# NVIDIA-Genomics-Research/GenomeWorks

Measured on AMD Instinct MI355X. Metric: cudapoa consensus GCUPS, 1024-window short-read batch (static band 256, 32 reads <= 1024 bp), higher is better.
Workload: dtype int16; 1 GPU; BASELINE configs[2]: cudapoa single-batch consensus, 1024 windows x 32 reads, backbone 960 bp, <=48 sub/24 ins/24 del, BatchConfig(1024,32,256,static_band), scores 8/-6/-8; windows_per_gpu=1024, cells_per_gpu=10990578176, parallelism=index-split x1

## Files before the change

### genomeworks_amd/csrc/poa_forward_moves.h

```cpp
#pragma once

namespace gwhip
{

constexpr int kKindShift = 60;
constexpr uint32_t kMoveHoriz = 1;

__device__ __forceinline__ uint32_t pk_mad_u16_vsv(uint32_t a, uint32_t s, uint32_t c)
{
    uint32_t d;
    asm("v_pk_mad_u16 %0, %1, %2, %3" : "=v"(d) : "v"(a), "s"(s), "v"(c));
    return d;
}
__device__ __forceinline__ uint32_t pk_mad_u16_vvs(uint32_t a, uint32_t b, uint32_t s)
{
    uint32_t d;
    asm("v_pk_mad_u16 %0, %1, %2, %3" : "=v"(d) : "v"(a), "v"(b), "s"(s));
    return d;
}
__device__ __forceinline__ void gstore_nt_u64(void* p, uint32_t lo, uint32_t hi)
{
    u32x2 v;
    v.x = lo; v.y = hi;
    __builtin_nontemporal_store(v, reinterpret_cast<u32x2*>(p));
}
__device__ __forceinline__ void gstore_u16_lane0_below(const void* vptr, uint32_t v)
{
    asm volatile("s_mov_b64 exec, 1\n\tglobal_store_short %0, %1, off offset:-2\n\ts_mov_b64 exec, -1" ::"v"(vptr), "v"(v) : "memory");
}

template <int MAXD = kPkMaxDist, bool TBRULES = false>
__device__ __forceinline__ int32_t classify_kinds(RowInfo<true>* rowinfo, int32_t graph_count, int lane, const uint64_t* xpred, int32_t dbg = 0)
{
    int32_t first_moved = graph_count + 1;
    for (int32_t r = 1 + lane; r <= graph_count; r += kWave)
    {
        RowInfo<true> ri  = rowinfo[r];
        const int32_t cnt = ri.cnt(), bs = ri.bs();
        uint64_t kind     = 4;
        const uint64_t xe  = (cnt > 3 && cnt <= 6 && xpred != nullptr) ? xpred[r & 255] : 0ull;
        const bool many_ok = cnt > 3 && cnt <= 6 && xpred_hit(xe, r, cnt) && !(dbg & (1 << 30));
        if (cnt >= 1 && (cnt <= 3 || many_ok))
        {
            bool ok    = true;
            int32_t d0 = 0, pbs0 = 0;
            for (int32_t k = 0; k < cnt; k++)
            {
                const int32_t p   = k < 3 ? ri.pred(k) : xpred_row(xe, k);
                const int32_t d   = r - p;
                const RowInfo<true> pri = rowinfo[p];
                const int32_t pbs = pri.bs();
                ok                = ok && d >= 1 && d <= MAXD && (bs - pbs) <= kPkGuardCols && (bs == 0 || pbs > 0);
                if constexpr (TBRULES) ok = ok && !(pri.cnt() == 0 && pbs > 0);
                if (k == 0) { d0 = d; pbs0 = pbs; }
            }
            if (ok) kind = cnt > 1 ? 3 : ((d0 == 1 && pbs0 == bs) ? 0 : ((d0 == 1 && bs - pbs0 == kCellsPerLane) ? 1 : 2));
        }
        if ((dbg & 1024) && kind <= 1) kind = 2;
        if ((dbg & 32768) && kind == 1) kind = 2;
        if ((dbg & 512) && (kind == 2 || kind == 3)) kind = 4;
        if ((dbg & 2048) && kind <= 1) kind = 4;
        ri.w       = (ri.w & ~(7ull << kKindShift)) | (kind << kKindShift);
        rowinfo[r] = ri;
        if (bs > 0) first_moved = min(first_moved, r);
    }
    for (int off = 32; off > 0; off >>= 1) first_moved = min(first_moved, __shfl_xor(first_moved, off));
    return __builtin_amdgcn_readfirstlane(first_moved);
}

constexpr uint64_t kRowScoresInHbm = 1ull << 63;
template <typename IdT>
__device__ __forceinline__ void mark_score_rows(const GraphView<IdT>& g, RowInfo<true>* rowinfo, int32_t graph_count, int lane, bool all_rows)
{
    auto mark = [&](int32_t row) {
        __hip_atomic_fetch_or(reinterpret_cast<uint32_t*>(&rowinfo[row].w) + 1, 0x80000000u, __ATOMIC_RELAXED, __HIP_MEMORY_SCOPE_WORKGROUP);
    };
    for (int32_t r = 1 + lane; r <= graph_count; r += kWave)
    {
        const uint64_t w    = rowinfo[r].w;
        const uint32_t kind = (uint32_t)(w >> kKindShift) & 7u;
        const int32_t cnt   = (int32_t)((w >> 8) & 0x3fu);
        const bool reads_or_recomputes = kind >= 4u || cnt > 3;
        if (reads_or_recomputes || ((w >> 14) & 1u) != 0 || all_rows) mark(r);
        if (reads_or_recomputes)
        {
            const int32_t node_id = cnt > 3 ? (int32_t)g.sorted_poa[r - 1] : 0;
            for (int32_t k = 0; k < cnt; k++)
                mark(k < 3 ? (int32_t)((w >> (24 + 12 * k)) & 0xfffu) : (int32_t)g.node_id_to_pos[g.incoming_edges[(int64_t)node_id * kEdges + k]] + 1);
        }
    }
    wave_sync();
}
__device__ __forceinline__ bool row_recompute_safe(uint64_t w)
{
    return ((uint32_t)(w >> kKindShift) & 7u) >= 4u || ((w >> 8) & 0x3fu) > 3u || ((w >> 15) & 0x1ffu) == 0u;
}

template <typename IdT, int BW>
__device__ __forceinline__ void banded_forward_moves(const GraphView<IdT>& g, RowInfo<true>* rowinfo, int32_t graph_count,
                                                     const uint8_t* lds_read, int16_t* scores, uint8_t* moves, uint8_t* ring,
                                                     const uint64_t* xpred, int32_t max_column, int32_t gap_score,
                                                     int32_t mismatch_score, int32_t match_score, int32_t dbg,
                                                     uint64_t* prof_acc, bool store_all = true)
{
    const bool abl       = (dbg & (1 << 14)) != 0;
    const bool st_scores = !(abl && (dbg & (1 << 26))), st_moves = !(abl && (dbg & (1 << 27)));
    const bool ab_ring = !(abl && (dbg & (1 << 20))), ab_guard = !(abl && (dbg & (1 << 19))), ab_scan = !(abl && (dbg & (1 << 18))),
               ab_moves = !(abl && (dbg & (1 << 17))), ab_rows = !(abl && (dbg & (1 << 16)));
    const int32_t ksel = prof_acc ? ((dbg >> 28) & 7) - 1 : -1;
    const bool kcount  = (dbg & (1 << 12)) != 0;
    uint64_t kacc      = 0;
    static_assert(BW == 128 || BW == 256, "band widths of the packed pass");
    constexpr int32_t band_width = BW;
    constexpr int32_t stride     = band_width + kRightPad;
    constexpr int kBandLanes     = BW / kCellsPerLane;
    const int lane               = threadIdx.x & (kWave - 1);
    const bool band_lane         = lane < kBandLanes;
    const int32_t lane4 = lane * 4, lane8 = lane * 8;
    const int32_t min_score = Limits<int16_t>::min / 2;

    const int32_t first_moved = classify_kinds(rowinfo, graph_count, lane, xpred, dbg);
    wave_sync();
    mark_score_rows<IdT>(g, rowinfo, graph_count, lane, store_all);

    const uint32_t MIN2   = pin_vgpr(pk_dup(min_score));
    const uint32_t SENT2  = pin_vgpr(pk_dup(kPkSentinel));
    const uint32_t GAP2   = pin_vgpr(pk_dup(gap_score));
    const uint32_t MAT2   = pin_vgpr(pk_dup(match_score));
    const uint32_t DIF2   = pin_vgpr(pk_dup(mismatch_score - match_score));
    const uint32_t ONE2   = pin_vgpr(0x00010001u);
    const uint32_t THREE2 = pin_vgpr(0x00030003u);
    const uint32_t NEG1   = pin_vgpr(0xffffffffu);
    const uint32_t K01 = pk_make((lane4 + 0) * gap_score, (lane4 + 1) * gap_score);
    const uint32_t K23 = pk_make((lane4 + 2) * gap_score, (lane4 + 3) * gap_score);
    const uint32_t ring_base = lds_addr(ring);
    const uint32_t read_base = lds_addr(lds_read);
    const uint32_t guard_off  = lane < 16 ? (uint32_t)(2 * BW) : (lane == 16 ? (uint32_t)-136 : (uint32_t)(120 - 16 * lane));
    const bool is_lane16      = lane == 16;
    const bool is_lane63      = lane == kBandLanes - 1;
    const uint32_t move_keep  = lane == 0 ? 0xffffff00u : 0xffffffffu;
    const uint32_t GUARD_HI_MIN = pin_vgpr(is_lane16 ? (((uint32_t)kPkSentinel & 0xffffu) | ((uint32_t)min_score << 16)) : pk_dup(kPkSentinel));
    const uint32_t S0X_MIN      = (uint32_t)min_score << 16;

    uint32_t P01 = pk_make((lane4 + 1) * gap_score, (lane4 + 2) * gap_score);
    uint32_t P23 = pk_make((lane4 + 3) * gap_score, (lane4 + 4) * gap_score);
    int32_t prev_rel0 = 0;
    uint32_t rd4  = lds_load_u32(read_base + lane4);
    uint32_t rd4n = lds_load_u32(read_base + lane4 + 4);
    uint32_t a1   = (uint32_t)lane8;
    uint32_t ga   = (a1 + guard_off) & (kPkSlotBytes - 1);
    uint8_t* const score_base = reinterpret_cast<uint8_t*>(scores) + lane8 + 2 * (1 + kRelShift);
    uint8_t* move_ptr  = moves + lane4 + (1 + kRelShift);

    if (BW == 256 || band_lane) lds_store_u64(ring_base + a1, P01, P23);
    lds_store_guard(ring_base + ga, SENT2, is_lane16 ? (((uint32_t)kPkSentinel & 0xffffu) | (0u << 16)) : SENT2);

    auto scan_row = [&](uint32_t s01, uint32_t s23, int32_t cu) {
        const uint32_t u01 = pk_sub(s01, K01), u23 = pk_sub(s23, K23);
        const uint32_t pm01 = pk_max(u01, (u01 << 16) | 0x8000u);
        const uint32_t pm23 = pk_max(u23, (u23 << 16) | 0x8000u);
        const int32_t m3    = (int32_t)pk_max(pm01, pm23) >> 16;
        const int32_t incl  = ab_scan ? wave_inclusive_max(m3) : m3;
        const int32_t excl  = max(wave_shr1(incl, cu), cu);
        const uint32_t ex2  = __builtin_amdgcn_perm((uint32_t)excl, (uint32_t)excl, 0x01000100u);
        const uint32_t m1b  = __builtin_amdgcn_perm(pm01, pm01, 0x03020302u);
        P01 = pk_add(pk_max(pm01, ex2), K01);
        P23 = pk_add(pk_max(pk_max(pm23, m1b), ex2), K23);
    };
    auto nz = [&](uint32_t a, uint32_t b) -> uint32_t { return pk_min_u16(pk_sub(a, b), ONE2); };
    auto costs = [&](uint32_t base4, uint32_t& c01, uint32_t& c23) {
        const uint32_t x   = rd4 ^ base4;
        const uint32_t x01 = __builtin_amdgcn_perm(0u, x, 0x0c010c00u);
        const uint32_t x23 = __builtin_amdgcn_perm(0u, x, 0x0c030c02u);
        c01 = pk_mad_u16(pk_min_u16(x01, ONE2), DIF2, MAT2);
        c23 = pk_mad_u16(pk_min_u16(x23, ONE2), DIF2, MAT2);
    };
    auto from_pred = [&](uint32_t s0x, uint32_t q01, uint32_t q23, uint32_t c01, uint32_t c23, uint32_t& D01, uint32_t& D23,
                         uint32_t& V01, uint32_t& V23) {
        D01 = pk_add(__builtin_amdgcn_alignbit(q01, s0x, 16), c01);
        D23 = pk_add(__builtin_amdgcn_alignbit(q23, q01, 16), c23);
        V01 = pk_add(q01, GAP2);
        V23 = pk_add(q23, GAP2);
    };
    auto store_row = [&](auto bs0_tag, int32_t r, int32_t rel0_val, uint32_t mv4, bool scores_to_hbm) {
        constexpr bool BS0 = decltype(bs0_tag)::value;
        move_ptr += stride;
        const uint32_t sbase = ring_base + (((uint32_t)r & (kPkSlots - 1)) * kPkSlotBytes);
        if (BS0 || __builtin_expect(scores_to_hbm, 0))
        {
            uint8_t* score_ptr = score_base + (uint32_t)r * (uint32_t)(stride * 2);
            if (st_scores && (BW == 256 || band_lane)) gstore_nt_u64(score_ptr, P01, P23);
            if constexpr (BS0) gstore_u16_lane0_below(score_ptr, (uint32_t)rel0_val);
        }
        if (ab_ring && (BW == 256 || band_lane)) lds_store_u64(sbase + a1, P01, P23);
        if constexpr (BS0)
        {
            const uint32_t rel0pk = ((uint32_t)kPkSentinel & 0xffffu) | ((uint32_t)rel0_val << 16);
            if (ab_guard) lds_store_guard(sbase + ga, SENT2, is_lane16 ? rel0pk : SENT2);
            prev_rel0 = rel0_val;
        }
        else if (ab_guard)
            lds_store_guard(sbase + ga, SENT2, GUARD_HI_MIN);
        if (st_moves && (BW == 256 || band_lane)) *reinterpret_cast<uint32_t*>(move_ptr) = mv4;
    };
    auto pack_moves = [&](uint32_t m01, uint32_t m23) -> uint32_t {
        return __builtin_amdgcn_perm(m23, m01, 0x06040200u) & move_keep;
    };

    auto general_row = [&](int32_t r, int32_t& prev_rel0_io) {
        const RowInfo<true> ri = uniform_row(rowinfo[r]);
        const int32_t bs       = ri.bs();
        const uint32_t base    = (uint32_t)ri.base();
        const int32_t prev_bs  = r > 1 ? uniform_row(rowinfo[r - 1]).bs() : 0;
        a1   = (uint32_t)(2 * bs + lane8) & (kPkSlotBytes - 1);
        ga   = (a1 + guard_off) & (kPkSlotBytes - 1);
        rd4  = lds_load_u32(read_base + bs + lane4);
        rd4n = lds_load_u32(read_base + bs + lane4 + 4);
        const int32_t pred_count = ri.cnt();
        const int32_t c          = bs + lane4;
        const int32_t cp0 = ((rd4 & 0xff) == base) ? match_score : mismatch_score;
        const int32_t cp1 = (((rd4 >> 8) & 0xff) == base) ? match_score : mismatch_score;
        const int32_t cp2 = (((rd4 >> 16) & 0xff) == base) ? match_score : mismatch_score;
        const int32_t cp3 = ((rd4 >> 24) == base) ? match_score : mismatch_score;
        const int32_t R0 = pk_lo(P01), R1 = pk_hi(P01), R2 = pk_lo(P23), R3 = pk_hi(P23);
        bool synced = false;
        auto from_regs = [&](int32_t& t0, int32_t& t1, int32_t& t2, int32_t& t3) {
            const int32_t q    = (bs - prev_bs) >> 2;
            const int32_t pend = min(prev_bs + band_width - kCellsPerLane, max_column);
            const int src      = lane + q;
            const int32_t from_left = __shfl(R3, src - 1);
            const int32_t S0        = (q == 0 && lane == 0) ? prev_rel0_io : from_left;
            const int32_t S1 = __shfl(R0, src), S2 = __shfl(R1, src), S3 = __shfl(R2, src), S4 = __shfl(R3, src);
            const bool valid = c <= pend;
            t0 = valid ? max(S0 + cp0, S1 + gap_score) : min_score;
            t1 = valid ? max(S1 + cp1, S2 + gap_score) : min_score;
            t2 = valid ? max(S2 + cp2, S3 + gap_score) : min_score;
            t3 = valid ? max(S3 + cp3, S4 + gap_score) : min_score;
        };
        auto from_hbm = [&](int32_t prow, int32_t& t0, int32_t& t1, int32_t& t2, int32_t& t3) {
            const int32_t pbs  = prow == 0 ? 0 : uniform_row(rowinfo[prow]).bs();
            const int32_t pend = min(pbs + band_width - kCellsPerLane, max_column);
            const bool valid   = !(c > pend || c < pbs);
            if (!synced) { wave_sync(); synced = true; }
            const int16_t* rowp = scores + (int64_t)prow * stride + (valid ? (c - pbs) : 0) + kRelShift;
            int32_t S0 = rowp[0];
            const Quad<int16_t> qd = *reinterpret_cast<const Quad<int16_t>*>(rowp + 1);
            const int32_t S1 = qd.v[0], S2 = qd.v[1], S3 = qd.v[2], S4 = qd.v[3];
            if (pbs > 0 && c == pbs) S0 = min_score;
            t0 = valid ? max(S0 + cp0, S1 + gap_score) : min_score;
            t1 = valid ? max(S1 + cp1, S2 + gap_score) : min_score;
            t2 = valid ? max(S2 + cp2, S3 + gap_score) : min_score;
            t3 = valid ? max(S3 + cp3, S4 + gap_score) : min_score;
        };
        auto rel0_of = [&](int32_t prow) -> int32_t {
            if (prow == r - 1) return prev_rel0_io;
            const int32_t pbs = prow == 0 ? 0 : uniform_row(rowinfo[prow]).bs();
            if (pbs > 0) return min_score;
            if (!synced) { wave_sync(); synced = true; }
            return wave_first((int32_t)scores[(int64_t)prow * stride + kRelShift]);
        };
        const int32_t node_id = (pred_count > 3) ? (int32_t)g.sorted_poa[r - 1] : 0;
        auto pred_row = [&](int32_t p) -> int32_t {
            if (pred_count == 0) return 0;
            if (p < 3) return ri.pred(p);
            return wave_first((int32_t)g.node_id_to_pos[g.incoming_edges[(int64_t)node_id * kEdges + p]] + 1);
        };
        int32_t fe = 0, rel0_val = min_score;
        if (pred_count == 0)
        {
            if (bs == 0) rel0_val = gap_score;
        }
        else
        {
            if (bs > kCellsPerLane && pred_count == 1)
                fe = min_score + gap_score;
            else
            {
                int32_t penalty = min_score;
                for (int32_t p = 0; p < pred_count; p++) penalty = max(penalty, rel0_of(pred_row(p)));
                fe = penalty + gap_score;
            }
            if (bs == 0) rel0_val = fe;
        }
        int32_t s0 = 0, s1 = 0, s2 = 0, s3 = 0;
        const int32_t np = max(pred_count, 1);
        for (int32_t p = 0; p < np; p++)
        {
            const int32_t prow = pred_row(p);
            int32_t t0, t1, t2, t3;
            if (prow == r - 1) from_regs(t0, t1, t2, t3);
            else from_hbm(prow, t0, t1, t2, t3);
            if (p == 0) { s0 = t0; s1 = t1; s2 = t2; s3 = t3; }
            else { s0 = max(s0, t0); s1 = max(s1, t1); s2 = max(s2, t2); s3 = max(s3, t3); }
        }
        scan_row(pk_make(s0, s1), pk_make(s2, s3), fe + gap_score);
        uint8_t* score_ptr = score_base + (uint32_t)r * (uint32_t)(stride * 2);
        move_ptr += stride;
        const uint32_t sbase  = ring_base + (((uint32_t)r & (kPkSlots - 1)) * kPkSlotBytes);
        const uint32_t rel0pk = ((uint32_t)kPkSentinel & 0xffffu) | ((uint32_t)rel0_val << 16);
        if (BW == 256 || band_lane)
        {
            *reinterpret_cast<uint2*>(score_ptr) = make_uint2(P01, P23);
            lds_store_u64(sbase + a1, P01, P23);
        }
        lds_store_guard(sbase + ga, SENT2, is_lane16 ? rel0pk : SENT2);
        if (bs == 0) gstore_u16_lane0_below(score_ptr, (uint32_t)rel0_val);
        if (BW == 256 || band_lane) *reinterpret_cast<uint32_t*>(move_ptr) = 0u;
        prev_rel0_io = rel0_val;
    };

    auto reg_row = [&](auto bs0_tag, auto moved_tag, int32_t r, uint32_t d0, uint32_t base4, bool scores_to_hbm) {
        constexpr bool BS0   = decltype(bs0_tag)::value;
        constexpr bool MOVED = decltype(moved_tag)::value;
        uint32_t s0x, q01, q23;
        if constexpr (!MOVED)
        {
            s0x = (uint32_t)wave_shr1((int32_t)P23, BS0 ? (int32_t)((uint32_t)prev_rel0 << 16) : (int32_t)S0X_MIN);
            q01 = P01; q23 = P23;
        }
        else
        {
            s0x  = P23;
            q01  = (uint32_t)wave_shl1((int32_t)P01, (int32_t)pk_dup(kPkSentinel));
            q23  = (uint32_t)wave_shl1((int32_t)P23, (int32_t)pk_dup(kPkSentinel));
            a1   = (a1 + 8) & (kPkSlotBytes - 1);
            ga   = (ga + 8) & (kPkSlotBytes - 1);
            rd4  = rd4n;
            rd4n = lds_load_u32(read_base + (((d0 >> 3) & 0x1ffu) << 2) + lane4 + 4);
        }
        int32_t cu = min_score + 2 * gap_score, rel0_val = min_score;
        if constexpr (BS0)
        {
            rel0_val = max(min_score, prev_rel0) + gap_score;
            cu       = rel0_val + gap_score;
        }
        uint32_t c01, c23, D01, D23, V01, V23;
        costs(base4, c01, c23);
        from_pred(s0x, q01, q23, c01, c23, D01, D23, V01, V23);
        uint32_t s01 = pk_max(D01, V01), s23 = pk_max(D23, V23);
        if constexpr (MOVED)
        {
            s01 = is_lane63 ? MIN2 : s01;
            s23 = is_lane63 ? MIN2 : s23;
        }
        scan_row(s01, s23, cu);
        const uint32_t m01 = pk_mad_u16(nz(P01, D01), pk_mad_u16(nz(P01, V01), NEG1, NEG1), THREE2);
        const uint32_t m23 = pk_mad_u16(nz(P23, D23), pk_mad_u16(nz(P23, V23), NEG1, NEG1), THREE2);
        uint32_t mv4 = ab_moves ? pack_moves(m01, m23) : 0u;
        if constexpr (MOVED) mv4 = is_lane63 ? 0u : mv4;
        store_row(bs0_tag, r, rel0_val, mv4, scores_to_hbm);
    };

    auto run_rows = [&](auto bs0_tag, int32_t r_from, int32_t r_to) {
        constexpr bool BS0 = decltype(bs0_tag)::value;
        int32_t r = r_from;
        while (r <= r_to)
        {
            const int32_t r0   = r;
            uint32_t D0v, D1v;
            {
                const int32_t rr    = min(r0 + lane, graph_count);
                const uint64_t w    = rowinfo[rr].w;
                const uint32_t kind = (uint32_t)(w >> kKindShift) & 7u;
                const uint32_t cnt  = (uint32_t)(w >> 8) & 0x3fu;
                const uint32_t bs4  = (uint32_t)(w >> 15) & 0x1ffu;
                const uint32_t p0 = (uint32_t)(w >> 24) & 0xfffu, p1 = (uint32_t)(w >> 36) & 0xfffu, p2 = (uint32_t)(w >> 48) & 0xfffu;
                const uint32_t slots = (p0 & 7u) | ((p1 & 7u) << 3) | ((p2 & 7u) << 6);
                const uint32_t dists = (((uint32_t)rr - p0) & 7u) | ((((uint32_t)rr - p1) & 7u) << 3) | ((((uint32_t)rr - p2) & 7u) << 6);
                D0v = kind | (bs4 << 3) | (slots << 12) | (dists << 21) | ((cnt <= 3 ? cnt : 0u) << 30);
                D1v = ((uint32_t)w & 0xffu) * 0x01010101u;
            }
            D0v = (r0 + lane <= r_to) ? D0v : 7u;
            const uint64_t need64 = BS0 ? ~0ull : __ballot((rowinfo[min(r0 + lane, graph_count)].w & kRowScoresInHbm) != 0);
            int32_t k      = 0;
            uint32_t d0    = (uint32_t)__builtin_amdgcn_readlane((int32_t)D0v, 0);
            uint32_t base4 = (uint32_t)__builtin_amdgcn_readlane((int32_t)D1v, 0);
            uint32_t kind  = d0 & 7u;
            auto advance = [&]() {
                r++;
                k++;
                const uint32_t nd = (uint32_t)__builtin_amdgcn_readlane((int32_t)D0v, k & (kWave - 1));
                base4 = (uint32_t)__builtin_amdgcn_readlane((int32_t)D1v, k & (kWave - 1));
                d0    = k == kWave ? 7u : nd;
                kind  = d0 & 7u;
            };
            for (;;)
            {
                const uint64_t t_k0 = ksel == 0 ? clock64() : 0;
                const int32_t r_k0  = r;
                while (kind == 0)
                {
                    reg_row(bs0_tag, std::false_type{}, r, d0, base4, ((need64 >> k) & 1ull) != 0);
                    advance();
                }
                if (ksel == 0) kacc += kcount ? (uint64_t)(r - r_k0) : clock64() - t_k0;
                if (kind == 7u) break;
                const int32_t kind_now = (int32_t)min(kind, 4u);
                const uint64_t t_kx    = ksel == kind_now ? clock64() : 0;
                const bool scores_to_hbm = ((need64 >> k) & 1ull) != 0;
                if (kind == 1)
                    reg_row(bs0_tag, std::true_type{}, r, d0, base4, scores_to_hbm);
                else if (kind <= 3)
                {
                    const uint32_t bs = ((d0 >> 3) & 0x1ffu) << 2;
                    a1 = (2u * bs + (uint32_t)lane8) & (kPkSlotBytes - 1);
                    ga = (a1 + guard_off) & (kPkSlotBytes - 1);
                    const uint32_t a0 = (a1 - 4) & (kPkSlotBytes - 1);
                    const uint32_t b0 = ring_base + (((d0 >> 12) & 7u) * kPkSlotBytes);
                    const uint32_t sent16 = (uint32_t)kPkSentinel & 0xffffu;
                    const uint32_t dd0 = (d0 >> 21) & 7u;
                    if (kind == 2)
                    {
                        const uint32_t x0 = lds_load_u32(b0 + a0);
                        const uint2 q0    = lds_load_u64(b0 + a1);
                        rd4  = lds_load_u32(read_base + bs + lane4);
                        rd4n = lds_load_u32(read_base + bs + lane4 + 4);
                        int32_t cu = min_score + 2 * gap_score, rel0_val = min_score;
                        if constexpr (BS0)
                        {
                            rel0_val = max(min_score, (int32_t)(int16_t)wave_first((int32_t)(lds_load_u32(b0 + kPkSlotBytes - 4) >> 16))) + gap_score;
                            cu       = rel0_val + gap_score;
                        }
                        uint32_t c01, c23, D01, D23, V01, V23;
                        costs(base4, c01, c23);
                        from_pred(x0, q0.x, q0.y, c01, c23, D01, D23, V01, V23);
                        const bool outside = (q0.x & 0xffffu) == sent16;
                        const uint32_t s01 = pk_max(D01, V01), s23 = pk_max(D23, V23);
                        scan_row(outside ? MIN2 : s01, outside ? MIN2 : s23, cu);
                        const uint32_t cD = pk_dup((int32_t)(2u * dd0 + 1u)), cV = pk_dup(1 - (int32_t)(2u * dd0));
                        const uint32_t m01 = pk_mad_u16_vvs(nz(P01, D01), pk_mad_u16_vsv(nz(P01, V01), cV, NEG1), cD);
                        const uint32_t m23 = pk_mad_u16_vvs(nz(P23, D23), pk_mad_u16_vsv(nz(P23, V23), cV, NEG1), cD);
                        const uint32_t mv4 = outside ? 0u : pack_moves(m01, m23);
                        store_row(bs0_tag, r, rel0_val, mv4, scores_to_hbm);
                    }
                    else
                    {
                        const uint32_t cnt3    = d0 >> 30;
                        const int32_t cnt      = cnt3 == 2 ? 2 : 3;
                        const uint32_t b1 = ring_base + (((d0 >> 15) & 7u) * kPkSlotBytes);
                        const uint32_t b2 = cnt > 2 ? ring_base + (((d0 >> 18) & 7u) * kPkSlotBytes) : b0;
                        const uint32_t dd1 = (d0 >> 24) & 7u, dd2 = (d0 >> 27) & 7u;
                        const uint32_t x0 = lds_load_u32(b0 + a0);
                        const uint2 q0    = lds_load_u64(b0 + a1);
                        const uint32_t x1 = lds_load_u32(b1 + a0);
                        const uint2 q1    = lds_load_u64(b1 + a1);
                        uint32_t x2 = 0;
                        uint2 q2 = make_uint2(0, 0);
                        if (cnt > 2)
                        {
                            x2 = lds_load_u32(b2 + a0);
                            q2 = lds_load_u64(b2 + a1);
                        }
                        rd4  = lds_load_u32(read_base + bs + lane4);
                        rd4n = lds_load_u32(read_base + bs + lane4 + 4);
                        int32_t fe = min_score + gap_score;
                        if constexpr (BS0)
                        {
                            int32_t pen = max(min_score, (int32_t)(int16_t)wave_first((int32_t)(lds_load_u32(b0 + kPkSlotBytes - 4) >> 16)));
                            pen = max(pen, (int32_t)(int16_t)wave_first((int32_t)(lds_load_u32(b1 + kPkSlotBytes - 4) >> 16)));
                            if (cnt > 2) pen = max(pen, (int32_t)(int16_t)wave_first((int32_t)(lds_load_u32(b2 + kPkSlotBytes - 4) >> 16)));
                            fe = pen + gap_score;
                        }
                        uint32_t c01, c23;
                        costs(base4, c01, c23);
                        uint32_t D0a, D0b, V0a, V0b, D1a, D1b, V1a, V1b;
                        from_pred(x0, q0.x, q0.y, c01, c23, D0a, D0b, V0a, V0b);
                        from_pred(x1, q1.x, q1.y, c01, c23, D1a, D1b, V1a, V1b);
                        const bool out0 = (q0.x & 0xffffu) == sent16, out1 = (q1.x & 0xffffu) == sent16;
                        bool undecided  = out0 | out1;
                        D0a = out0 ? MIN2 : D0a; D0b = out0 ? MIN2 : D0b; V0a = out0 ? MIN2 : V0a; V0b = out0 ? MIN2 : V0b;
                        D1a = out1 ? MIN2 : D1a; D1b = out1 ? MIN2 : D1b; V1a = out1 ? MIN2 : V1a; V1b = out1 ? MIN2 : V1b;
                        uint32_t bD01 = pk_max(D0a, D1a), bD23 = pk_max(D0b, D1b), bV01 = pk_max(V0a, V1a), bV23 = pk_max(V0b, V1b);
                        const uint32_t mD0 = pk_dup((int32_t)(2u * dd0 + 1u)), mV0 = pk_dup((int32_t)(2u * dd0));
                        const uint32_t E1  = pk_dup(2 * ((int32_t)dd1 - (int32_t)dd0));
                        uint32_t A01, A23, B01, B23;
                        if (cnt > 2)
                        {
                            uint32_t D2a, D2b, V2a, V2b;
                            from_pred(x2, q2.x, q2.y, c01, c23, D2a, D2b, V2a, V2b);
                            const bool out2 = (q2.x & 0xffffu) == sent16;
                            undecided       = undecided | out2;
                            D2a = out2 ? MIN2 : D2a; D2b = out2 ? MIN2 : D2b; V2a = out2 ? MIN2 : V2a; V2b = out2 ? MIN2 : V2b;
                            bD01 = pk_max(bD01, D2a); bD23 = pk_max(bD23, D2b); bV01 = pk_max(bV01, V2a); bV23 = pk_max(bV23, V2b);
                            const uint32_t E2  = pin_vgpr(pk_dup(2 * ((int32_t)dd2 - (int32_t)dd1)));
                            const uint32_t E1v = pin_vgpr(E1);
                            A01 = pk_mad_u16_vvs(nz(bD01, D0a), pk_mad_u16(nz(bD01, D1a), E2, E1v), mD0);
                            A23 = pk_mad_u16_vvs(nz(bD23, D0b), pk_mad_u16(nz(bD23, D1b), E2, E1v), mD0);
                            B01 = pk_mad_u16_vvs(nz(bV01, V0a), pk_mad_u16(nz(bV01, V1a), E2, E1v), mV0);
                            B23 = pk_mad_u16_vvs(nz(bV23, V0b), pk_mad_u16(nz(bV23, V1b), E2, E1v), mV0);
                        }
                        else
                        {
                            const uint32_t E1v = pin_vgpr(E1);
                            A01 = pk_mad_u16_vvs(nz(bD01, D0a), E1v, mD0); A23 = pk_mad_u16_vvs(nz(bD23, D0b), E1v, mD0);
                            B01 = pk_mad_u16_vvs(nz(bV01, V0a), E1v, mV0); B23 = pk_mad_u16_vvs(nz(bV23, V0b), E1v, mV0);
                        }
                        if (cnt3 == 0)
                        {
                            const uint64_t xe     = wave_first64(xpred[r & 255]);
                            const int32_t cnt_all = (int32_t)((xe >> 13) & 63u);
                            uint32_t xD01 = MIN2, xD23 = MIN2, xV01 = MIN2, xV23 = MIN2;
                            int32_t pen_x = min_score;
                            for (int32_t kk = 3; kk < cnt_all; kk++)
                            {
                                const uint32_t bk = ring_base + (((uint32_t)xpred_row(xe, kk) & 7u) * kPkSlotBytes);
                                const uint32_t xk = lds_load_u32(bk + a0);
                                const uint2 qk    = lds_load_u64(bk + a1);
                                uint32_t Da, Db, Va, Vb;
                                from_pred(xk, qk.x, qk.y, c01, c23, Da, Db, Va, Vb);
                                const bool outk = (qk.x & 0xffffu) == sent16;
                                undecided       = undecided | outk;
                                xD01 = pk_max(xD01, outk ? MIN2 : Da); xD23 = pk_max(xD23, outk ? MIN2 : Db);
                                xV01 = pk_max(xV01, outk ? MIN2 : Va); xV23 = pk_max(xV23, outk ? MIN2 : Vb);
                                if constexpr (BS0) pen_x = max(pen_x, (int32_t)(int16_t)wave_first((int32_t)(lds_load_u32(bk + kPkSlotBytes - 4) >> 16)));
                            }
                            if constexpr (BS0) fe = max(fe - gap_score, pen_x) + gap_score;
                            const uint32_t fD01 = pk_max(bD01, xD01), fD23 = pk_max(bD23, xD23), fV01 = pk_max(bV01, xV01), fV23 = pk_max(bV23, xV23);
                            A01 = pk_mad_u16(nz(bD01, fD01), pk_sub(0u, A01), A01); A23 = pk_mad_u16(nz(bD23, fD23), pk_sub(0u, A23), A23);
                            B01 = pk_mad_u16(nz(bV01, fV01), pk_sub(0u, B01), B01); B23 = pk_mad_u16(nz(bV23, fV23), pk_sub(0u, B23), B23);
                            bD01 = fD01; bD23 = fD23; bV01 = fV01; bV23 = fV23;
                        }
                        const int32_t rel0_val = BS0 ? fe : min_score;
                        scan_row(pk_max(bD01, bV01), pk_max(bD23, bV23), fe + gap_score);
                        auto move_of = [&](uint32_t H, uint32_t bD, uint32_t bV, uint32_t A, uint32_t B) -> uint32_t {
                            const uint32_t t1 = pk_mad_u16(nz(H, bV), pk_sub(ONE2, B), B);
                            return pk_mad_u16(nz(H, bD), pk_sub(t1, A), A);
                        };
                        const uint32_t m01 = move_of(P01, bD01, bV01, A01, B01);
                        const uint32_t m23 = move_of(P23, bD23, bV23, A23, B23);
                        const uint32_t mv4 = undecided ? 0u : pack_moves(m01, m23);
                        store_row(bs0_tag, r, rel0_val, mv4, scores_to_hbm);
                    }
                }
                else
                {
                    general_row(r, prev_rel0);
                    if constexpr (!BS0) prev_rel0 = min_score;
                }
                if (ksel == kind_now) kacc += kcount ? 1 : clock64() - t_kx;
                advance();
            }
        }
    };

    const int32_t bs0_end = min(first_moved - 1, graph_count);
    if (!ab_rows) return;
    run_rows(std::true_type{}, 1, bs0_end);
    run_rows(std::false_type{}, bs0_end + 1, graph_count);
    if (ksel >= 0 && lane == 0) *prof_acc += kacc;
}

}
```

Measured before the change: 394.4 GCUPS.

## Precompute per-row operand descriptors per wave block and dispatch rows via readlane

Row metadata for a block of 63 rows is now decoded once into per-lane operand records: ring slot addresses, band-shift offset, read address, move-code multipliers, and flag bits for the dispatch. The row loop then fetches these with readlane instead of recomputing slot addresses and move constants per row. Ring rows are split into a templated handler specialised by predecessor count. The move pointer becomes an indexed address instead of a running increment. The aim is to cut scalar decode work and branching in the inner row loop, at the cost of more VGPRs for the operand record.

```diff
diff --git a/genomeworks_amd/csrc/poa_forward_moves.h b/genomeworks_amd/csrc/poa_forward_moves.h
--- a/genomeworks_amd/csrc/poa_forward_moves.h
+++ b/genomeworks_amd/csrc/poa_forward_moves.h
@@ -1,4 +1,6 @@
 #pragma once
+
+#include "poa_forward_row_operands.h"
 
 namespace gwhip
 {
@@ -33,13 +35,14 @@
 __device__ __forceinline__ int32_t classify_kinds(RowInfo<true>* rowinfo, int32_t graph_count, int lane, const uint64_t* xpred, int32_t dbg = 0)
 {
     int32_t first_moved = graph_count + 1;
+    const bool demote_many = (dbg & (1 << 30)) != 0 && (dbg & (1 << 13)) == 0;
     for (int32_t r = 1 + lane; r <= graph_count; r += kWave)
     {
         RowInfo<true> ri  = rowinfo[r];
         const int32_t cnt = ri.cnt(), bs = ri.bs();
         uint64_t kind     = 4;
         const uint64_t xe  = (cnt > 3 && cnt <= 6 && xpred != nullptr) ? xpred[r & 255] : 0ull;
-        const bool many_ok = cnt > 3 && cnt <= 6 && xpred_hit(xe, r, cnt) && !(dbg & (1 << 30));
+        const bool many_ok = cnt > 3 && cnt <= 6 && xpred_hit(xe, r, cnt) && !demote_many;
         if (cnt >= 1 && (cnt <= 3 || many_ok))
         {
             bool ok    = true;
@@ -108,8 +111,14 @@
     const bool ab_ring = !(abl && (dbg & (1 << 20))), ab_guard = !(abl && (dbg & (1 << 19))), ab_scan = !(abl && (dbg & (1 << 18))),
                ab_moves = !(abl && (dbg & (1 << 17))), ab_rows = !(abl && (dbg & (1 << 16)));
     const int32_t ksel = prof_acc ? ((dbg >> 28) & 7) - 1 : -1;
+    const bool kfine   = (dbg & (1 << 13)) != 0;
     const bool kcount  = (dbg & (1 << 12)) != 0;
     uint64_t kacc      = 0;
+    auto kselected = [&](uint32_t dk) -> bool { return ksel == (int32_t)((kfine || dk < kDkRingThree) ? dk : (uint32_t)kDkRingTwo); };
+    const bool ksel_prev = kselected(kDkPrev), ksel_moved = kselected(kDkPrevMoved), ksel_one = kselected(kDkRingOne),
+               ksel_two = kselected(kDkRingTwo), ksel_three = kselected(kDkRingThree), ksel_many = kselected(kDkRingMany),
+               ksel_general = kselected(kDkGeneral);
+    static_assert(kRowOpSlots == kPkSlots && kRowOpSlotBytes == kPkSlotBytes, "the row operands fold the ring's geometry in");
     static_assert(BW == 128 || BW == 256, "band widths of the packed pass");
     constexpr int32_t band_width = BW;
     constexpr int32_t stride     = band_width + kRightPad;
@@ -150,7 +159,7 @@
     uint32_t a1   = (uint32_t)lane8;
     uint32_t ga   = (a1 + guard_off) & (kPkSlotBytes - 1);
     uint8_t* const score_base = reinterpret_cast<uint8_t*>(scores) + lane8 + 2 * (1 + kRelShift);
-    uint8_t* move_ptr  = moves + lane4 + (1 + kRelShift);
+    uint8_t* const move_base  = moves + lane4 + (1 + kRelShift);
 
     if (BW == 256 || band_lane) lds_store_u64(ring_base + a1, P01, P23);
     lds_store_guard(ring_base + ga, SENT2, is_lane16 ? (((uint32_t)kPkSentinel & 0xffffu) | (0u << 16)) : SENT2);
@@ -184,7 +193,6 @@
     };
     auto store_row = [&](auto bs0_tag, int32_t r, int32_t rel0_val, uint32_t mv4, bool scores_to_hbm) {
         constexpr bool BS0 = decltype(bs0_tag)::value;
-        move_ptr += stride;
         const uint32_t sbase = ring_base + (((uint32_t)r & (kPkSlots - 1)) * kPkSlotBytes);
         if (BS0 || __builtin_expect(scores_to_hbm, 0))
         {
@@ -201,7 +209,7 @@
         }
         else if (ab_guard)
             lds_store_guard(sbase + ga, SENT2, GUARD_HI_MIN);
-        if (st_moves && (BW == 256 || band_lane)) *reinterpret_cast<uint32_t*>(move_ptr) = mv4;
+        if (st_moves && (BW == 256 || band_lane)) *reinterpret_cast<uint32_t*>(move_base + (uint32_t)r * (uint32_t)stride) = mv4;
     };
     auto pack_moves = [&](uint32_t m01, uint32_t m23) -> uint32_t {
         return __builtin_amdgcn_perm(m23, m01, 0x06040200u) & move_keep;
@@ -295,7 +303,6 @@
         }
         scan_row(pk_make(s0, s1), pk_make(s2, s3), fe + gap_score);
         uint8_t* score_ptr = score_base + (uint32_t)r * (uint32_t)(stride * 2);
-        move_ptr += stride;
         const uint32_t sbase  = ring_base + (((uint32_t)r & (kPkSlots - 1)) * kPkSlotBytes);
         const uint32_t rel0pk = ((uint32_t)kPkSentinel & 0xffffu) | ((uint32_t)rel0_val << 16);
         if (BW == 256 || band_lane)
@@ -305,7 +312,7 @@
         }
         lds_store_guard(sbase + ga, SENT2, is_lane16 ? rel0pk : SENT2);
         if (bs == 0) gstore_u16_lane0_below(score_ptr, (uint32_t)rel0_val);
-        if (BW == 256 || band_lane) *reinterpret_cast<uint32_t*>(move_ptr) = 0u;
+        if (BW == 256 || band_lane) *reinterpret_cast<uint32_t*>(move_base + (uint32_t)r * (uint32_t)stride) = 0u;
         prev_rel0_io = rel0_val;
     };
 
@@ -326,7 +333,7 @@
             a1   = (a1 + 8) & (kPkSlotBytes - 1);
             ga   = (ga + 8) & (kPkSlotBytes - 1);
             rd4  = rd4n;
-            rd4n = lds_load_u32(read_base + (((d0 >> 3) & 0x1ffu) << 2) + lane4 + 4);
+            rd4n = lds_load_u32((d0 >> kRowOpReadShift) + lane4 + 4);
         }
         int32_t cu = min_score + 2 * gap_score, rel0_val = min_score;
         if constexpr (BS0)
@@ -351,195 +358,203 @@
         store_row(bs0_tag, r, rel0_val, mv4, scores_to_hbm);
     };
 
+    auto ring_row = [&](auto bs0_tag, auto np_tag, int32_t r, int32_t k, uint32_t d0, uint32_t base4, const RowOperands& OPv) {
+        constexpr bool BS0 = decltype(bs0_tag)::value;
+        constexpr int NP   = decltype(np_tag)::value;
+        auto fetch = [&](uint32_t v) -> uint32_t { return (uint32_t)__builtin_amdgcn_readlane((int32_t)v, k); };
+        const uint32_t b0 = fetch(OPv.slot0), bs2 = fetch(OPv.bs2), m0 = fetch(OPv.mv0), m1 = fetch(OPv.mv1);
+        const uint32_t b1 = NP >= 2 ? fetch(OPv.slot1) : 0u, m2 = NP >= 2 ? fetch(OPv.mv2) : 0u;
+        const uint32_t b2 = NP >= 3 ? fetch(OPv.slot2) : 0u, m3 = NP >= 3 ? fetch(OPv.mv3) : 0u;
+        const uint32_t rdb = (d0 >> kRowOpReadShift) + (uint32_t)lane4;
+        const bool scores_to_hbm = (d0 & kRowOpScoresToHbm) != 0;
+        a1 = (bs2 + (uint32_t)lane8) & (kPkSlotBytes - 1);
+        ga = (a1 + guard_off) & (kPkSlotBytes - 1);
+        const uint32_t a0     = (a1 - 4) & (kPkSlotBytes - 1);
+        const uint32_t sent16 = (uint32_t)kPkSentinel & 0xffffu;
+        auto rel0_in = [&](uint32_t b) -> int32_t { return (int32_t)(int16_t)wave_first((int32_t)(lds_load_u32(b + kPkSlotBytes - 4) >> 16)); };
+        if constexpr (NP == 1)
+        {
+            const uint32_t x0 = lds_load_u32(b0 + a0);
+            const uint2 q0    = lds_load_u64(b0 + a1);
+            rd4  = lds_load_u32(rdb);
+            rd4n = lds_load_u32(rdb + 4);
+            int32_t cu = min_score + 2 * gap_score, rel0_val = min_score;
+            if constexpr (BS0)
+            {
+                rel0_val = max(min_score, rel0_in(b0)) + gap_score;
+                cu       = rel0_val + gap_score;
+            }
+            uint32_t c01, c23, D01, D23, V01, V23;
+            costs(base4, c01, c23);
+            from_pred(x0, q0.x, q0.y, c01, c23, D01, D23, V01, V23);
+            const bool outside = (q0.x & 0xffffu) == sent16;
+            const uint32_t s01 = pk_max(D01, V01), s23 = pk_max(D23, V23);
+            scan_row(outside ? MIN2 : s01, outside ? MIN2 : s23, cu);
+            const uint32_t m01 = pk_mad_u16_vvs(nz(P01, D01), pk_mad_u16_vsv(nz(P01, V01), m1, NEG1), m0);
+            const uint32_t m23 = pk_mad_u16_vvs(nz(P23, D23), pk_mad_u16_vsv(nz(P23, V23), m1, NEG1), m0);
+            const uint32_t mv4 = outside ? 0u : pack_moves(m01, m23);
+            store_row(bs0_tag, r, rel0_val, mv4, scores_to_hbm);
+        }
+        else
+        {
+            const uint32_t x0 = lds_load_u32(b0 + a0);
+            const uint2 q0    = lds_load_u64(b0 + a1);
+            const uint32_t x1 = lds_load_u32(b1 + a0);
+            const uint2 q1    = lds_load_u64(b1 + a1);
+            uint32_t x2 = 0;
+            uint2 q2 = make_uint2(0, 0);
+            if constexpr (NP > 2)
+            {
+                x2 = lds_load_u32(b2 + a0);
+                q2 = lds_load_u64(b2 + a1);
+            }
+            rd4  = lds_load_u32(rdb);
+            rd4n = lds_load_u32(rdb + 4);
+            int32_t fe = min_score + gap_score;
+            if constexpr (BS0)
+            {
+                int32_t pen = max(min_score, rel0_in(b0));
+                pen = max(pen, rel0_in(b1));
+                if constexpr (NP > 2) pen = max(pen, rel0_in(b2));
+                fe = pen + gap_score;
+            }
+            uint32_t c01, c23;
+            costs(base4, c01, c23);
+            uint32_t D0a, D0b, V0a, V0b, D1a, D1b, V1a, V1b;
+            from_pred(x0, q0.x, q0.y, c01, c23, D0a, D0b, V0a, V0b);
+            from_pred(x1, q1.x, q1.y, c01, c23, D1a, D1b, V1a, V1b);
+            const bool out0 = (q0.x & 0xffffu) == sent16, out1 = (q1.x & 0xffffu) == sent16;
+            bool undecided  = out0 | out1;
+            D0a = out0 ? MIN2 : D0a; D0b = out0 ? MIN2 : D0b; V0a = out0 ? MIN2 : V0a; V0b = out0 ? MIN2 : V0b;
+            D1a = out1 ? MIN2 : D1a; D1b = out1 ? MIN2 : D1b; V1a = out1 ? MIN2 : V1a; V1b = out1 ? MIN2 : V1b;
+            uint32_t bD01 = pk_max(D0a, D1a), bD23 = pk_max(D0b, D1b), bV01 = pk_max(V0a, V1a), bV23 = pk_max(V0b, V1b);
+            const uint32_t E1v = pin_vgpr(m2);
+            uint32_t A01, A23, B01, B23;
+            if constexpr (NP > 2)
+            {
+                uint32_t D2a, D2b, V2a, V2b;
+                from_pred(x2, q2.x, q2.y, c01, c23, D2a, D2b, V2a, V2b);
+                const bool out2 = (q2.x & 0xffffu) == sent16;
+                undecided       = undecided | out2;
+                D2a = out2 ? MIN2 : D2a; D2b = out2 ? MIN2 : D2b; V2a = out2 ? MIN2 : V2a; V2b = out2 ? MIN2 : V2b;
+                bD01 = pk_max(bD01, D2a); bD23 = pk_max(bD23, D2b); bV01 = pk_max(bV01, V2a); bV23 = pk_max(bV23, V2b);
+                const uint32_t E2 = pin_vgpr(m3);
+                A01 = pk_mad_u16_vvs(nz(bD01, D0a), pk_mad_u16(nz(bD01, D1a), E2, E1v), m0);
+                A23 = pk_mad_u16_vvs(nz(bD23, D0b), pk_mad_u16(nz(bD23, D1b), E2, E1v), m0);
+                B01 = pk_mad_u16_vvs(nz(bV01, V0a), pk_mad_u16(nz(bV01, V1a), E2, E1v), m1);
+                B23 = pk_mad_u16_vvs(nz(bV23, V0b), pk_mad_u16(nz(bV23, V1b), E2, E1v), m1);
+            }
+            else
+            {
+                A01 = pk_mad_u16_vvs(nz(bD01, D0a), E1v, m0); A23 = pk_mad_u16_vvs(nz(bD23, D0b), E1v, m0);
+                B01 = pk_mad_u16_vvs(nz(bV01, V0a), E1v, m1); B23 = pk_mad_u16_vvs(nz(bV23, V0b), E1v, m1);
+            }
+            if constexpr (NP > 3)
+            {
+                const uint64_t xe     = wave_first64(xpred[r & 255]);
+                const int32_t cnt_all = (int32_t)((xe >> 13) & 63u);
+                uint32_t xD01 = MIN2, xD23 = MIN2, xV01 = MIN2, xV23 = MIN2;
+                int32_t pen_x = min_score;
+                for (int32_t kk = 3; kk < cnt_all; kk++)
+                {
+                    const uint32_t bk = ring_base + (((uint32_t)xpred_row(xe, kk) & 7u) * kPkSlotBytes);
+                    const uint32_t xk = lds_load_u32(bk + a0);
+                    const uint2 qk    = lds_load_u64(bk + a1);
+                    uint32_t Da, Db, Va, Vb;
+                    from_pred(xk, qk.x, qk.y, c01, c23, Da, Db, Va, Vb);
+                    const bool outk = (qk.x & 0xffffu) == sent16;
+                    undecided       = undecided | outk;
+                    xD01 = pk_max(xD01, outk ? MIN2 : Da); xD23 = pk_max(xD23, outk ? MIN2 : Db);
+                    xV01 = pk_max(xV01, outk ? MIN2 : Va); xV23 = pk_max(xV23, outk ? MIN2 : Vb);
+                    if constexpr (BS0) pen_x = max(pen_x, rel0_in(bk));
+                }
+                if constexpr (BS0) fe = max(fe - gap_score, pen_x) + gap_score;
+                const uint32_t fD01 = pk_max(bD01, xD01), fD23 = pk_max(bD23, xD23), fV01 = pk_max(bV01, xV01), fV23 = pk_max(bV23, xV23);
+                A01 = pk_mad_u16(nz(bD01, fD01), pk_sub(0u, A01), A01); A23 = pk_mad_u16(nz(bD23, fD23), pk_sub(0u, A23), A23);
+                B01 = pk_mad_u16(nz(bV01, fV01), pk_sub(0u, B01), B01); B23 = pk_mad_u16(nz(bV23, fV23), pk_sub(0u, B23), B23);
+                bD01 = fD01; bD23 = fD23; bV01 = fV01; bV23 = fV23;
+            }
+            const int32_t rel0_val = BS0 ? fe : min_score;
+            scan_row(pk_max(bD01, bV01), pk_max(bD23, bV23), fe + gap_score);
+            auto move_of = [&](uint32_t H, uint32_t bD, uint32_t bV, uint32_t A, uint32_t B) -> uint32_t {
+                const uint32_t t1 = pk_mad_u16(nz(H, bV), pk_sub(ONE2, B), B);
+                return pk_mad_u16(nz(H, bD), pk_sub(t1, A), A);
+            };
+            const uint32_t m01 = move_of(P01, bD01, bV01, A01, B01);
+            const uint32_t m23 = move_of(P23, bD23, bV23, A23, B23);
+            const uint32_t mv4 = undecided ? 0u : pack_moves(m01, m23);
+            store_row(bs0_tag, r, rel0_val, mv4, scores_to_hbm);
+        }
+    };
+
+    constexpr int32_t kBlockRows = kWave - 1;
     auto run_rows = [&](auto bs0_tag, int32_t r_from, int32_t r_to) {
         constexpr bool BS0 = decltype(bs0_tag)::value;
+        const uint64_t kone = !kfine ? 1ull : (BS0 ? 1ull << 32 : 1ull << 48);
         int32_t r = r_from;
         while (r <= r_to)
         {
-            const int32_t r0   = r;
-            uint32_t D0v, D1v;
-            {
-                const int32_t rr    = min(r0 + lane, graph_count);
-                const uint64_t w    = rowinfo[rr].w;
-                const uint32_t kind = (uint32_t)(w >> kKindShift) & 7u;
-                const uint32_t cnt  = (uint32_t)(w >> 8) & 0x3fu;
-                const uint32_t bs4  = (uint32_t)(w >> 15) & 0x1ffu;
-                const uint32_t p0 = (uint32_t)(w >> 24) & 0xfffu, p1 = (uint32_t)(w >> 36) & 0xfffu, p2 = (uint32_t)(w >> 48) & 0xfffu;
-                const uint32_t slots = (p0 & 7u) | ((p1 & 7u) << 3) | ((p2 & 7u) << 6);
-                const uint32_t dists = (((uint32_t)rr - p0) & 7u) | ((((uint32_t)rr - p1) & 7u) << 3) | ((((uint32_t)rr - p2) & 7u) << 6);
-                D0v = kind | (bs4 << 3) | (slots << 12) | (dists << 21) | ((cnt <= 3 ? cnt : 0u) << 30);
-                D1v = ((uint32_t)w & 0xffu) * 0x01010101u;
-            }
-            D0v = (r0 + lane <= r_to) ? D0v : 7u;
-            const uint64_t need64 = BS0 ? ~0ull : __ballot((rowinfo[min(r0 + lane, graph_count)].w & kRowScoresInHbm) != 0);
-            int32_t k      = 0;
-            uint32_t d0    = (uint32_t)__builtin_amdgcn_readlane((int32_t)D0v, 0);
-            uint32_t base4 = (uint32_t)__builtin_amdgcn_readlane((int32_t)D1v, 0);
-            uint32_t kind  = d0 & 7u;
-            auto advance = [&]() {
-                r++;
+            const int32_t rr     = min(r + lane, graph_count);
+            const RowOperands OPv = pack_row_operands(rowinfo[rr].w, (uint32_t)rr, lane < kBlockRows && r + lane <= r_to, ring_base, read_base);
+            const int32_t r0 = r;
+            int32_t k        = 0;
+            uint32_t d0, base4;
+            auto fetch = [&]() {
+                d0    = (uint32_t)__builtin_amdgcn_readlane((int32_t)OPv.d0, k);
+                base4 = (uint32_t)__builtin_amdgcn_readlane((int32_t)OPv.base4, k);
+            };
+            auto timed = [&](auto dk_tag, bool selected, auto&& body) {
+                const uint64_t t = selected ? clock64() : 0;
+                body();
+                if (selected) kacc += kcount ? kone : clock64() - t;
                 k++;
-                const uint32_t nd = (uint32_t)__builtin_amdgcn_readlane((int32_t)D0v, k & (kWave - 1));
-                base4 = (uint32_t)__builtin_amdgcn_readlane((int32_t)D1v, k & (kWave - 1));
-                d0    = k == kWave ? 7u : nd;
-                kind  = d0 & 7u;
+                asm volatile("; end of a row of kind %0" ::"n"(decltype(dk_tag)::value));
             };
             for (;;)
             {
-                const uint64_t t_k0 = ksel == 0 ? clock64() : 0;
-                const int32_t r_k0  = r;
-                while (kind == 0)
-                {
-                    reg_row(bs0_tag, std::false_type{}, r, d0, base4, ((need64 >> k) & 1ull) != 0);
-                    advance();
-                }
-                if (ksel == 0) kacc += kcount ? (uint64_t)(r - r_k0) : clock64() - t_k0;
-                if (kind == 7u) break;
-                const int32_t kind_now = (int32_t)min(kind, 4u);
-                const uint64_t t_kx    = ksel == kind_now ? clock64() : 0;
-                const bool scores_to_hbm = ((need64 >> k) & 1ull) != 0;
-                if (kind == 1)
-                    reg_row(bs0_tag, std::true_type{}, r, d0, base4, scores_to_hbm);
-                else if (kind <= 3)
-                {
-                    const uint32_t bs = ((d0 >> 3) & 0x1ffu) << 2;
-                    a1 = (2u * bs + (uint32_t)lane8) & (kPkSlotBytes - 1);
-                    ga = (a1 + guard_off) & (kPkSlotBytes - 1);
-                    const uint32_t a0 = (a1 - 4) & (kPkSlotBytes - 1);
-                    const uint32_t b0 = ring_base + (((d0 >> 12) & 7u) * kPkSlotBytes);
-                    const uint32_t sent16 = (uint32_t)kPkSentinel & 0xffffu;
-                    const uint32_t dd0 = (d0 >> 21) & 7u;
-                    if (kind == 2)
-                    {
-                        const uint32_t x0 = lds_load_u32(b0 + a0);
-                        const uint2 q0    = lds_load_u64(b0 + a1);
-                        rd4  = lds_load_u32(read_base + bs + lane4);
-                        rd4n = lds_load_u32(read_base + bs + lane4 + 4);
-                        int32_t cu = min_score + 2 * gap_score, rel0_val = min_score;
-                        if constexpr (BS0)
-                        {
-                            rel0_val = max(min_score, (int32_t)(int16_t)wave_first((int32_t)(lds_load_u32(b0 + kPkSlotBytes - 4) >> 16))) + gap_score;
-                            cu       = rel0_val + gap_score;
-                        }
-                        uint32_t c01, c23, D01, D23, V01, V23;
-                        costs(base4, c01, c23);
-                        from_pred(x0, q0.x, q0.y, c01, c23, D01, D23, V01, V23);
-                        const bool outside = (q0.x & 0xffffu) == sent16;
-                        const uint32_t s01 = pk_max(D01, V01), s23 = pk_max(D23, V23);
-                        scan_row(outside ? MIN2 : s01, outside ? MIN2 : s23, cu);
-                        const uint32_t cD = pk_dup((int32_t)(2u * dd0 + 1u)), cV = pk_dup(1 - (int32_t)(2u * dd0));
-                        const uint32_t m01 = pk_mad_u16_vvs(nz(P01, D01), pk_mad_u16_vsv(nz(P01, V01), cV, NEG1), cD);
-                        const uint32_t m23 = pk_mad_u16_vvs(nz(P23, D23), pk_mad_u16_vsv(nz(P23, V23), cV, NEG1), cD);
-                        const uint32_t mv4 = outside ? 0u : pack_moves(m01, m23);
-                        store_row(bs0_tag, r, rel0_val, mv4, scores_to_hbm);
-                    }
-                    else
-                    {
-                        const uint32_t cnt3    = d0 >> 30;
-                        const int32_t cnt      = cnt3 == 2 ? 2 : 3;
-                        const uint32_t b1 = ring_base + (((d0 >> 15) & 7u) * kPkSlotBytes);
-                        const uint32_t b2 = cnt > 2 ? ring_base + (((d0 >> 18) & 7u) * kPkSlotBytes) : b0;
-                        const uint32_t dd1 = (d0 >> 24) & 7u, dd2 = (d0 >> 27) & 7u;
-                        const uint32_t x0 = lds_load_u32(b0 + a0);
-                        const uint2 q0    = lds_load_u64(b0 + a1);
-                        const uint32_t x1 = lds_load_u32(b1 + a0);
-                        const uint2 q1    = lds_load_u64(b1 + a1);
-                        uint32_t x2 = 0;
-                        uint2 q2 = make_uint2(0, 0);
-                        if (cnt > 2)
-                        {
-                            x2 = lds_load_u32(b2 + a0);
-                            q2 = lds_load_u64(b2 + a1);
-                        }
-                        rd4  = lds_load_u32(read_base + bs + lane4);
-                        rd4n = lds_load_u32(read_base + bs + lane4 + 4);
-                        int32_t fe = min_score + gap_score;
-                        if constexpr (BS0)
-                        {
-                            int32_t pen = max(min_score, (int32_t)(int16_t)wave_first((int32_t)(lds_load_u32(b0 + kPkSlotBytes - 4) >> 16)));
-                            pen = max(pen, (int32_t)(int16_t)wave_first((int32_t)(lds_load_u32(b1 + kPkSlotBytes - 4) >> 16)));
-                            if (cnt > 2) pen = max(pen, (int32_t)(int16_t)wave_first((int32_t)(lds_load_u32(b2 + kPkSlotBytes - 4) >> 16)));
-                            fe = pen + gap_score;
-                        }
-                        uint32_t c01, c23;
-                        costs(base4, c01, c23);
-                        uint32_t D0a, D0b, V0a, V0b, D1a, D1b, V1a, V1b;
-                        from_pred(x0, q0.x, q0.y, c01, c23, D0a, D0b, V0a, V0b);
-                        from_pred(x1, q1.x, q1.y, c01, c23, D1a, D1b, V1a, V1b);
-                        const bool out0 = (q0.x & 0xffffu) == sent16, out1 = (q1.x & 0xffffu) == sent16;
-                        bool undecided  = out0 | out1;
-                        D0a = out0 ? MIN2 : D0a; D0b = out0 ? MIN2 : D0b; V0a = out0 ? MIN2 : V0a; V0b = out0 ? MIN2 : V0b;
-                        D1a = out1 ? MIN2 : D1a; D1b = out1 ? MIN2 : D1b; V1a = out1 ? MIN2 : V1a; V1b = out1 ? MIN2 : V1b;
-                        uint32_t bD01 = pk_max(D0a, D1a), bD23 = pk_max(D0b, D1b), bV01 = pk_max(V0a, V1a), bV23 = pk_max(V0b, V1b);
-                        const uint32_t mD0 = pk_dup((int32_t)(2u * dd0 + 1u)), mV0 = pk_dup((int32_t)(2u * dd0));
-                        const uint32_t E1  = pk_dup(2 * ((int32_t)dd1 - (int32_t)dd0));
-                        uint32_t A01, A23, B01, B23;
-                        if (cnt > 2)
-                        {
-                            uint32_t D2a, D2b, V2a, V2b;
-                            from_pred(x2, q2.x, q2.y, c01, c23, D2a, D2b, V2a, V2b);
-                            const bool out2 = (q2.x & 0xffffu) == sent16;
-                            undecided       = undecided | out2;
-                            D2a = out2 ? MIN2 : D2a; D2b = out2 ? MIN2 : D2b; V2a = out2 ? MIN2 : V2a; V2b = out2 ? MIN2 : V2b;
-                            bD01 = pk_max(bD01, D2a); bD23 = pk_max(bD23, D2b); bV01 = pk_max(bV01, V2a); bV23 = pk_max(bV23, V2b);
-                            const uint32_t E2  = pin_vgpr(pk_dup(2 * ((int32_t)dd2 - (int32_t)dd1)));
-                            const uint32_t E1v = pin_vgpr(E1);
-                            A01 = pk_mad_u16_vvs(nz(bD01, D0a), pk_mad_u16(nz(bD01, D1a), E2, E1v), mD0);
-                            A23 = pk_mad_u16_vvs(nz(bD23, D0b), pk_mad_u16(nz(bD23, D1b), E2, E1v), mD0);
-                            B01 = pk_mad_u16_vvs(nz(bV01, V0a), pk_mad_u16(nz(bV01, V1a), E2, E1v), mV0);
-                            B23 = pk_mad_u16_vvs(nz(bV23, V0b), pk_mad_u16(nz(bV23, V1b), E2, E1v), mV0);
-                        }
-                        else
-                        {
-                            const uint32_t E1v = pin_vgpr(E1);
-                            A01 = pk_mad_u16_vvs(nz(bD01, D0a), E1v, mD0); A23 = pk_mad_u16_vvs(nz(bD23, D0b), E1v, mD0);
-                            B01 = pk_mad_u16_vvs(nz(bV01, V0a), E1v, mV0); B23 = pk_mad_u16_vvs(nz(bV23, V0b), E1v, mV0);
-                        }
-                        if (cnt3 == 0)
-                        {
-                            const uint64_t xe     = wave_first64(xpred[r & 255]);
-                            const int32_t cnt_all = (int32_t)((xe >> 13) & 63u);
-                            uint32_t xD01 = MIN2, xD23 = MIN2, xV01 = MIN2, xV23 = MIN2;
-                            int32_t pen_x = min_score;
-                            for (int32_t kk = 3; kk < cnt_all; kk++)
-                            {
-                                const uint32_t bk = ring_base + (((uint32_t)xpred_row(xe, kk) & 7u) * kPkSlotBytes);
-                                const uint32_t xk = lds_load_u32(bk + a0);
-                                const uint2 qk    = lds_load_u64(bk + a1);
-                                uint32_t Da, Db, Va, Vb;
-                                from_pred(xk, qk.x, qk.y, c01, c23, Da, Db, Va, Vb);
-                                const bool outk = (qk.x & 0xffffu) == sent16;
-                                undecided       = undecided | outk;
-                                xD01 = pk_max(xD01, outk ? MIN2 : Da); xD23 = pk_max(xD23, outk ? MIN2 : Db);
-                                xV01 = pk_max(xV01, outk ? MIN2 : Va); xV23 = pk_max(xV23, outk ? MIN2 : Vb);
-                                if constexpr (BS0) pen_x = max(pen_x, (int32_t)(int16_t)wave_first((int32_t)(lds_load_u32(bk + kPkSlotBytes - 4) >> 16)));
-                            }
-                            if constexpr (BS0) fe = max(fe - gap_score, pen_x) + gap_score;
-                            const uint32_t fD01 = pk_max(bD01, xD01), fD23 = pk_max(bD23, xD23), fV01 = pk_max(bV01, xV01), fV23 = pk_max(bV23, xV23);
-                            A01 = pk_mad_u16(nz(bD01, fD01), pk_sub(0u, A01), A01); A23 = pk_mad_u16(nz(bD23, fD23), pk_sub(0u, A23), A23);
-                            B01 = pk_mad_u16(nz(bV01, fV01), pk_sub(0u, B01), B01); B23 = pk_mad_u16(nz(bV23, fV23), pk_sub(0u, B23), B23);
-                            bD01 = fD01; bD23 = fD23; bV01 = fV01; bV23 = fV23;
-                        }
-                        const int32_t rel0_val = BS0 ? fe : min_score;
-                        scan_row(pk_max(bD01, bV01), pk_max(bD23, bV23), fe + gap_score);
-                        auto move_of = [&](uint32_t H, uint32_t bD, uint32_t bV, uint32_t A, uint32_t B) -> uint32_t {
-                            const uint32_t t1 = pk_mad_u16(nz(H, bV), pk_sub(ONE2, B), B);
-                            return pk_mad_u16(nz(H, bD), pk_sub(t1, A), A);
-                        };
-                        const uint32_t m01 = move_of(P01, bD01, bV01, A01, B01);
-                        const uint32_t m23 = move_of(P23, bD23, bV23, A23, B23);
-                        const uint32_t mv4 = undecided ? 0u : pack_moves(m01, m23);
-                        store_row(bs0_tag, r, rel0_val, mv4, scores_to_hbm);
-                    }
-                }
-                else
-                {
-                    general_row(r, prev_rel0);
+                fetch();
+                const uint64_t t_k0 = ksel_prev ? clock64() : 0;
+                const int32_t k_k0  = k;
+                while ((d0 & 7u) == kDkPrev)
+                {
+                    reg_row(bs0_tag, std::false_type{}, r0 + k, d0, base4, (d0 & kRowOpScoresToHbm) != 0);
+                    k++;
+                    fetch();
+                }
+                if (ksel_prev) kacc += kcount ? (uint64_t)(k - k_k0) * kone : clock64() - t_k0;
+                if (d0 & kRowOpIsRingTwo)
+                {
+                    timed(std::integral_constant<uint32_t, kDkRingTwo>{}, ksel_two, [&]() { ring_row(bs0_tag, std::integral_constant<int, 2>{}, r0 + k, k, d0, base4, OPv); });
+                    continue;
+                }
+                if (d0 & kRowOpIsRingOne)
+                {
+                    timed(std::integral_constant<uint32_t, kDkRingOne>{}, ksel_one, [&]() { ring_row(bs0_tag, std::integral_constant<int, 1>{}, r0 + k, k, d0, base4, OPv); });
+                    continue;
+                }
+                if (d0 & kRowOpIsPrevMoved)
+                {
+                    timed(std::integral_constant<uint32_t, kDkPrevMoved>{}, ksel_moved, [&]() { reg_row(bs0_tag, std::true_type{}, r0 + k, d0, base4, (d0 & kRowOpScoresToHbm) != 0); });
+                    continue;
+                }
+                if (d0 & kRowOpIsEnd) break;
+                const uint32_t kind = d0 & 7u;
+                if (kind == kDkRingThree)
+                {
+                    timed(std::integral_constant<uint32_t, kDkRingThree>{}, ksel_three, [&]() { ring_row(bs0_tag, std::integral_constant<int, 3>{}, r0 + k, k, d0, base4, OPv); });
+                    continue;
+                }
+                if (kind == kDkRingMany)
+                {
+                    timed(std::integral_constant<uint32_t, kDkRingMany>{}, ksel_many, [&]() { ring_row(bs0_tag, std::integral_constant<int, 4>{}, r0 + k, k, d0, base4, OPv); });
+                    continue;
+                }
+                timed(std::integral_constant<uint32_t, kDkGeneral>{}, ksel_general, [&]() {
+                    general_row(r0 + k, prev_rel0);
                     if constexpr (!BS0) prev_rel0 = min_score;
-                }
-                if (ksel == kind_now) kacc += kcount ? 1 : clock64() - t_kx;
-                advance();
-            }
+                });
+            }
+            r = r0 + k;
         }
     };
 
diff --git a/genomeworks_amd/csrc/poa_forward_row_operands.h b/genomeworks_amd/csrc/poa_forward_row_operands.h
--- /dev/null
+++ b/genomeworks_amd/csrc/poa_forward_row_operands.h
@@ -0,0 +1,62 @@
+#pragma once
+
+#include <cstdint>
+
+#if defined(__HIPCC__)
+#define GWHIP_ROW_OPERANDS_FN __host__ __device__ inline
+#else
+#define GWHIP_ROW_OPERANDS_FN inline
+#endif
+
+namespace gwhip
+{
+
+constexpr uint32_t kDkPrev = 0, kDkPrevMoved = 1, kDkRingOne = 2, kDkRingTwo = 3, kDkGeneral = 4, kDkRingThree = 5, kDkRingMany = 6,
+                   kDkEnd = 7;
+constexpr uint32_t kRowOpSlots = 8, kRowOpSlotBytes = 1024;
+constexpr uint32_t kRowOpScoresToHbm = 1u << 3;
+constexpr uint32_t kRowOpIsRingTwo = 1u << 4, kRowOpIsRingOne = 1u << 5, kRowOpIsPrevMoved = 1u << 6, kRowOpIsEnd = 1u << 7;
+constexpr int kRowOpReadShift      = 8;
+
+struct RowOperands
+{
+    uint32_t d0;
+    uint32_t base4;
+    uint32_t slot0, slot1, slot2;
+    uint32_t bs2;
+    uint32_t mv0, mv1, mv2, mv3;
+};
+
+GWHIP_ROW_OPERANDS_FN uint32_t row_operand_dup16(int32_t v) { return ((uint32_t)v & 0xffffu) | ((uint32_t)v << 16); }
+
+GWHIP_ROW_OPERANDS_FN uint32_t row_descriptor_kind(uint32_t kind, uint32_t cnt)
+{
+    if (kind == 3u) return cnt == 2u ? kDkRingTwo : (cnt == 3u ? kDkRingThree : kDkRingMany);
+    return kind > 4u ? kDkGeneral : kind;
+}
+
+GWHIP_ROW_OPERANDS_FN RowOperands pack_row_operands(uint64_t w, uint32_t row, bool in_block, uint32_t ring_base, uint32_t read_base)
+{
+    const uint32_t kind = (uint32_t)(w >> 60) & 7u;
+    const uint32_t cnt  = (uint32_t)(w >> 8) & 0x3fu;
+    const uint32_t bs   = ((uint32_t)(w >> 15) & 0x1ffu) << 2;
+    const uint32_t p0 = (uint32_t)(w >> 24) & 0xfffu, p1 = (uint32_t)(w >> 36) & 0xfffu, p2 = (uint32_t)(w >> 48) & 0xfffu;
+    const int32_t dd0 = (int32_t)((row - p0) & 7u), dd1 = (int32_t)((row - p1) & 7u), dd2 = (int32_t)((row - p2) & 7u);
+    const uint32_t dk = in_block ? row_descriptor_kind(kind, cnt) : kDkEnd;
+    RowOperands o;
+    const uint32_t kind_bits = dk == kDkRingTwo ? kRowOpIsRingTwo : (dk == kDkRingOne ? kRowOpIsRingOne : (dk == kDkPrevMoved ? kRowOpIsPrevMoved : (dk == kDkEnd ? kRowOpIsEnd : 0u)));
+    o.d0    = dk | ((uint32_t)(w >> 63) << 3) | kind_bits | ((read_base + bs) << kRowOpReadShift);
+    o.base4 = ((uint32_t)w & 0xffu) * 0x01010101u;
+    o.slot0 = ring_base + (p0 & (kRowOpSlots - 1)) * kRowOpSlotBytes;
+    o.slot1 = ring_base + (p1 & (kRowOpSlots - 1)) * kRowOpSlotBytes;
+    o.slot2 = ring_base + (p2 & (kRowOpSlots - 1)) * kRowOpSlotBytes;
+    o.bs2   = 2u * bs;
+    const bool one = kind == kDkRingOne;
+    o.mv0 = row_operand_dup16(2 * dd0 + 1);
+    o.mv1 = row_operand_dup16(one ? 1 - 2 * dd0 : 2 * dd0);
+    o.mv2 = row_operand_dup16(2 * (dd1 - dd0));
+    o.mv3 = row_operand_dup16(2 * (dd2 - dd1));
+    return o;
+}
+
+}
```

After: 432.6 GCUPS, median of 6. 1.1x the previous value.
